# thanard/me-trpo

Measured on AMD Instinct MI355X. Metric: imagined env-steps/sec (KxBxH) over the full TRPO iteration, higher is better.
Workload: dtype f32

## Files before the change

### me-trpo_amd/_lib.py

```python
import ctypes as C
import os

import torch

_HERE = os.path.dirname(os.path.abspath(__file__))
LIB_PATH = os.path.join(_HERE, "libmetrpo.so")
MAX_LAYERS = 6

ENV_IDS = {'swimmer': 0, 'half_cheetah': 1, 'half-cheetah': 1, 'ant': 2, 'humanoid': 3, 'hopper': 4, 'snake': 5}
SAM_MODES = {'step_rand': 0, 'eps_rand': 1, 'model_mean_std': 2, 'model_mean': 3, 'model_med': 4, 'one_model': 5}
DYN_PRECISIONS = {'f32': 0, 'bf16': 1}
ACTS = {'identity': 0, 'tf.identity': 0, 'relu': 1, 'tf.nn.relu': 1, 'tanh': 2, 'tf.nn.tanh': 2, 'tf.tanh': 2}


class Dims(C.Structure):
    _fields_ = [('env', C.c_int32), ('ns', C.c_int32), ('na', C.c_int32), ('n_models', C.c_int32),
                ('dyn_n_hidden', C.c_int32), ('dyn_hidden', C.c_int32 * MAX_LAYERS), ('dyn_act', C.c_int32 * MAX_LAYERS),
                ('n_drop', C.c_int32), ('pol_n_hidden', C.c_int32), ('pol_hidden', C.c_int32 * MAX_LAYERS)]


class RolloutArgs(C.Structure):
    _fields_ = [('B', C.c_int32), ('T', C.c_int32), ('H', C.c_int32), ('sam_mode', C.c_int32), ('determ', C.c_int32),
                ('eval_all_heads', C.c_int32), ('d_pool', C.c_void_p), ('n_pool', C.c_int32), ('seed', C.c_uint64),
                ('stream_offset', C.c_uint64), ('d_eps', C.c_void_p), ('d_model_idx', C.c_void_p),
# ... 132 lines not shown
    'metrpo_bptt_grad_stochastic': (_I, [_P, _P, _I, _I, _D, _P, C.c_uint64, _P, _P, _P, _P]),
    'metrpo_set_exclusive': (_I, [_P, _I]),
    'metrpo_set_option': (_I, [_P, C.c_char_p, C.c_char_p]),
    'metrpo_get_option': (_I, [_P, C.c_char_p, C.c_char_p, _I]),
    'metrpo_option_name': (C.c_char_p, [_I]),
    'metrpo_last_rollout_kernel': (_I, [_P]),
    'metrpo_rollout_note': (C.c_char_p, [_P]),
    'metrpo_set_dyn_precision': (_I, [_P, _I]),
    'metrpo_get_dyn_precision': (_I, [_P]),
    'metrpo_policy_adam_reset': (_I, [_P, _P]),
    'metrpo_policy_adam_step': (_I, [_P, _P, _D, _D, _D, _D, _D, _P]),
    'metrpo_lbfgs_begin': (_I, [_P, _I, _P, C.POINTER(LbfgsOpts), _P, _P]),
    'metrpo_lbfgs_iterate': (_I, [_P, _P, _P, _P, _P, _P]),
    'metrpo_lbfgs_get_result': (_I, [_P, C.POINTER(LbfgsResult), _P]),
    'metrpo_lbfgs_policy': (_I, [_P, _P, _I, _I, _D, C.POINTER(LbfgsOpts), C.POINTER(LbfgsResult), _P]),
    'metrpo_get_dyn_adam': (_I, [_P, _P, _P, C.POINTER(_L), _P]),
    'metrpo_set_dyn_adam': (_I, [_P, _P, _P, _L, _P]),
    'metrpo_get_policy_adam': (_I, [_P, _P, _P, C.POINTER(_L), _P]),
    'metrpo_set_policy_adam': (_I, [_P, _P, _P, _L, _P]),
}
EXTRA_SYMBOLS = {
    'metrpo_rollout_generic': (_I, [_P, C.POINTER(RolloutArgs), _P]),
    'metrpo_has_mfma_path': (_I, [_P]),
    'metrpo_set_update_path': (_I, [_P, _I]),
    'metrpo_update_path': (_I, [_P, _L]),
    'metrpo_set_rollout_variant': (_I, [_P, _I]),
    'metrpo_set_det_path': (_I, [_P, _I]),
    'metrpo_probe_peaks': (_I, [_P, _P, _P]),
    'metrpo_schedulable_cus': (_I, [_P, _P]),
    'metrpo_debug_fvp_us': (_I, [_P, _P, _P]),
    'metrpo_debug_last_update': (_I, [_P, _P]),
    'metrpo_debug_persist_stats': (_I, [_P, _P, _I, _P]),
    'metrpo_debug_ws_retired': (_I, [_P, _P, _I]),
}


def load():
    if not os.path.exists(LIB_PATH):
        raise ImportError("libmetrpo.so not found at %s -- build it with `python -c 'import __graft_entry__ as g; "
                          "g.build()'` (hipcc --offload-arch=gfx950); there is no CPU fallback" % LIB_PATH)
    lib = C.CDLL(LIB_PATH)
    for table in (SYMBOLS, EXTRA_SYMBOLS):
        for name, (res, args) in table.items():
            fn = getattr(lib, name)
            fn.restype, fn.argtypes = res, args
    if lib.metrpo_abi_version() != 4:
        raise ImportError("libmetrpo.so ABI version mismatch")
    return lib


lib = load()


class MetrpoError(RuntimeError):
    pass


def check(rc, ctx=None):
    if rc != 0:
        msg = lib.metrpo_status_string(rc).decode()
        if ctx:
            msg += ": " + lib.metrpo_last_error(ctx).decode()
        raise MetrpoError(msg)
```

### me-trpo_amd/csrc/metrpo_internal.h

```cpp
#pragma once
#include <hip/hip_runtime.h>
#include <stdint.h>
#include <string>
#include <atomic>
#include <utility>
#include <vector>
#include "metrpo.h"
#include "xchg_device.h"

#define MAXL (METRPO_MAX_LAYERS + 1)
#define WAVE 64

struct NetDesc {
    int n_layers;
    int dims[MAXL + 1];
    int act[MAXL];
    int w_off[MAXL];
    int b_off[MAXL];
    int n_params;
    int api_w_off[MAXL];
    int api_b_off[MAXL];
    int api_n_params;
    int max_width;
};
// ... 48 lines not shown
    int rollout_variant = 0;
    DevBuf<float> d_partials;
    DevBuf<double> d_cg;
    DevBuf<float> d_vf;
    DevBuf<float> d_theta_try;
    DevBuf<double> d_valbuf;
    DevBuf<double> d_vbuf;
    DevBuf<double> d_gae_part;
    DevBuf<double> d_gram_part;
    DevBuf<unsigned int> d_ticket;
    DevBuf<float> d_hcache;
    DevBuf<void> d_sub;
    DevBuf<void> d_merr; DevBuf<double> d_merr_part;
    DevBuf<double> d_ppo_kl;
    DevBuf<void> d_mig; int mig_epoch = 0;
    void* nccl_comm = nullptr; int comm_world = 0, comm_rank = 0;
    void* xg_region = nullptr; void* xg_peer[XCHG_MAX_WORLD] = {}; int xg_world = 0, xg_rank = 0, xg_cap = 0; unsigned int xg_seq = 0; unsigned long long xg_timeout = 0;
    int pol_path = 1;
    DevBuf<void> d_pg; long long pg_fwd_rows = -1; const float* pg_fwd_obs = nullptr;
    int pol_f3 = 0;
    DevBuf<void> d_f3; long long f3_rows = -1; const float* f3_obs = nullptr; const float* f3_theta = nullptr; int f3_img_ok = 0;
    DevBuf<void> d_adam;
    long long adam_t = 0;
    DevBuf<void> d_train;
    DevBuf<double> d_train_part;
    DevBuf<void> d_big;
    DevBuf<void> d_res; unsigned int res_seq = 0;
    DevBuf<unsigned long long> d_skp_stats; int skp_stats_n = 0;
    std::vector<int> skp_tab_host;
    DevBuf<void> d_skp_tab; long long skp_key[8] = {-1, -1, -1, -1, -1, -1, -1, -1}; int skp_Jx[8] = {}, skp_Jmax = 0, skp_L = 0, skp_NSL = 0; int persist_failed = 0;
    int res_failed = 0;
    int last_ract_kernel = -1;
    DevBuf<int32_t> d_ract_model;
    int last_rollout_kernel = -1;
    int dyn_precision = METRPO_DYN_F32;
    DevBuf<uint16_t> d_dyn_bf16;
    double* h_upd = nullptr; unsigned long long upd_stamp = 0;
    DevBuf<double> d_lb; int lb_n = 0, lb_m = 0, lb_open = 0; double* h_lb = nullptr; unsigned long long lb_stamp = 0;
    int upd_pending = 0, upd_spec = 0, upd_changed_in_end = 0; metrpo_batch upd_batch = {}; metrpo_trpo_params upd_params = {}; metrpo_trpo_diag upd_diag = {};
    hipStream_t side_stream[METRPO_MAX_PAR_ROUNDS - 1] = {}; hipEvent_t ev_fork = nullptr, ev_join[METRPO_MAX_PAR_ROUNDS - 1] = {}; int side_ready = 0;
    double* h_pinned = nullptr;
    int n_sm = 256;
    int upd_tiles_per_wave = 1;
    int n_cu_sched = 0;
    int exclusive = 1;
    std::string opt_val[OPT_COUNT]; bool opt_set[OPT_COUNT] = {};
    hipEvent_t fvp_ev[32] = {}; int fvp_ev_n = 0, fvp_ev_made = 0;
    struct UpdLast { int family = -1, op = -1, table = -1, pt = 0, nrows = 0, splits = 0, kchunk = 0; } upd_last;
    std::string rollout_note;
    int fallback_logged = 0;
    std::vector<std::pair<void*, size_t>> ws_retired; size_t ws_retired_bytes = 0;
    std::string err;
};

constexpr size_t WS_RETIRED_MAX = (size_t)4 << 30;
static inline void ws_sweep(metrpo_ctx* c) {
    for (const auto& r : c->ws_retired) (void)hipFree(r.first);
    c->ws_retired.clear(); c->ws_retired_bytes = 0;
}
int set_err(metrpo_ctx* c, int code, const std::string& msg);
template <class T> static inline int ws_grow(metrpo_ctx* c, DevBuf<T>& b, size_t bytes, bool* grew = nullptr) {
    if (grew) *grew = false;
    if (bytes <= b.bytes) return METRPO_OK;
    if (b.p) {
        c->ws_retired.emplace_back((void*)b.p, b.bytes); c->ws_retired_bytes += b.bytes;
        b.p = nullptr; b.bytes = 0;
// ... 225 lines not shown
```

### me-trpo_amd/csrc/rollout_coop.hip

```cpp
#define COOP_MAIN_TU 1
#include "rollout_coop_kernel.h"

#define CENTRY_ENV(ENVID) CENTRY(ENVID, 5), CENTRY(ENVID, 4), CENTRY(ENVID, 3), CENTRY(ENVID, 2), CENTRY(ENVID, 1)
static const CoopEntry kCoop[] = {
    CENTRY_ENV(METRPO_ENV_SWIMMER), CENTRY_ENV(METRPO_ENV_HALF_CHEETAH), CENTRY_ENV(METRPO_ENV_HOPPER),
    CENTRY_ENV(METRPO_ENV_SNAKE), CENTRY_ENV(METRPO_ENV_ANT),
};
extern const CoopEntry kCoopK6[5], kCoopK7[5], kCoopK8[5], kCoopK9[5], kCoopK10[5];
constexpr int N_COOP = (int)(sizeof(kCoop) / sizeof(kCoop[0]));
static const CoopEntry& coop_entry(int idx) {
    if (idx < N_COOP) return kCoop[idx];
    const CoopEntry* wide[5] = {kCoopK6, kCoopK7, kCoopK8, kCoopK9, kCoopK10};
    return wide[(idx - N_COOP) / 5][(idx - N_COOP) % 5];
}

int coop_select_config(metrpo_ctx* c) {
    const ProblemDesc& pd = c->pd;
    if (mfma_shape_config(c) < 0 || pd.dyn.dims[1] != 64 || pd.dyn.dims[2] != 64 || pd.pol.dims[1] != 32 || pd.pol.dims[2] != 32) return -1;
    for (int i = 0; i < N_COOP + 25; ++i)
        if (coop_entry(i).env == pd.env && coop_entry(i).K == pd.K && coop_entry(i).kern[1][0] != nullptr) return i;
    return -1;
}

__global__ void __launch_bounds__(256) k_pad_dyn(NetDesc src, NetDesc dst, int K, const float* __restrict__ s, float* __restrict__ d) {
    const long long idx = (long long)blockIdx.x * 256 + threadIdx.x;
    if (idx >= (long long)K * dst.n_params) return;
    const int k = (int)(idx / dst.n_params), o = (int)(idx % dst.n_params);
    const float* sk = s + (size_t)k * src.n_params;
    float v = 0.0f;
    for (int l = 0; l < dst.n_layers; ++l) {
        const int din = dst.dims[l], dout = dst.dims[l + 1];
        if (o >= dst.w_off[l] && o < dst.w_off[l] + din * dout) {
            const int i = (o - dst.w_off[l]) / dout, j = (o - dst.w_off[l]) % dout;
            if (i < src.dims[l] && j < src.dims[l + 1]) v = sk[src.w_off[l] + i * src.dims[l + 1] + j];
        } else if (o >= dst.b_off[l] && o < dst.b_off[l] + dout) {
            const int j = o - dst.b_off[l];
            if (j < src.dims[l + 1]) v = sk[src.b_off[l] + j];
        }
    }
    d[idx] = v;
}

int launch_pad_dyn(metrpo_ctx* c, hipStream_t st) {
    const long long n = (long long)c->pd.K * c->dyn_pad.n_params;
    hipLaunchKernelGGL(k_pad_dyn, dim3((unsigned)((n + 255) / 256)), dim3(256), 0, st, c->pd.dyn, c->dyn_pad, c->pd.K, c->d_dyn.p, c->d_dyn_pad.p);
    HIP_TRY(c, hipGetLastError());
    return METRPO_OK;
}

int launch_rollout_coop(metrpo_ctx* c, int idx, const RolloutK& r_in, hipStream_t st, bool padded) {
    const CoopEntry& en = coop_entry(idx);
    const size_t sh = sizeof(float) * (size_t)en.lds_floats;
    const int tiles = (r_in.B + 15) / 16;
    RolloutK r = r_in;
    const int n_cu = (tiles > c->n_sm / 2) ? sched_cus(c, st) : c->n_sm;
    bool one = tiles <= n_cu || en.always_one;
    if (!one) {
        const long long slots = 2LL * n_cu, rounds = tiles / slots, rest = tiles % slots;
        const double t_one = (double)tiles / n_cu;
        const double t_two = en.pair * rounds + (rest == 0 ? 0.0 : rest <= n_cu ? 1.0 + en.rem_slope * (en.pair - 1.0) * rest / n_cu : en.pair);
        one = t_one < t_two;
    }
    if (c->rollout_variant == 2) one = false;
    if (one && tiles > n_cu && !ctx_exclusive(c)) one = false;
    if (!one && en.kern[0][0] == nullptr) return METRPO_EUNSUPPORTED;
    const int grid = one ? (tiles < n_cu ? tiles : n_cu) : tiles;
    if (one && tiles > grid) {
        const int ns = c->pd.ns;
        const size_t tile_bytes = sizeof(int32_t) * (1 + 32 + 16 * (size_t)ns);
        bool grew = false;
        { const int rc = ws_grow(c, c->d_mig, tile_bytes * (size_t)tiles, &grew); if (rc) return rc; }
        if (grew) { HIP_TRY(c, hipMemsetAsync(c->d_mig.p, 0, c->d_mig.bytes, st)); c->mig_epoch = 0; }
        const size_t cap = c->d_mig.bytes / tile_bytes;
        int32_t* base = (int32_t*)c->d_mig.p;
        r.mig_flag = base; r.mig_ts = base + cap; r.mig_model = base + 17 * cap;
        r.mig_obs = (float*)(base + 33 * cap);
        r.mig_epoch = ++c->mig_epoch;
        r.mig_err = comm_err_cell(c) + 1;
    }
    const bool draws = r.eps || r.model_idx || r.sel_noise || r.reset_idx || r.reset_model;
    const coop_kernel_t kern = en.kern[one ? 1 : 0][draws ? 1 : 0];
    if (sh > 64 * 1024) HIP_TRY(c, hipFuncSetAttribute((const void*)kern, hipFuncAttributeMaxDynamicSharedMemorySize, (int)sh));
    const float* dyn = c->d_dyn.p;
    if (padded) { const int rc = launch_pad_dyn(c, st); if (rc) return rc; dyn = c->d_dyn_pad.p; }
    hipLaunchKernelGGL(kern, dim3(grid), dim3(256), sh, st, r, dyn, c->d_theta.p, c->d_norm.p);
    HIP_TRY(c, hipGetLastError());
    return METRPO_OK;
}
```

### me-trpo_amd/csrc/rollout_coop_kernel.h

```cpp
#pragma once
#include "dyn_head_mfma.h"

#if defined(COOP_TIMING) && defined(COOP_MAIN_TU)
__device__ unsigned long long g_coop_phase[4][16];
#define PH_NOW() __builtin_readcyclecounter()
#define PH_DECL unsigned long long ph_t = PH_NOW(); unsigned long long ph_acc[14] = {0, 0, 0, 0, 0, 0, 0, 0, 0, 0, 0, 0, 0, 0};
#define PH_MARK(i) { if ((COOP_TIMING >> (i)) & 1) { const unsigned long long n_ = PH_NOW(); ph_acc[i] += n_ - ph_t; ph_t = n_; } }
#define PH_DUMP { if (lane == 0 && blockIdx.x == 0) for (int i_ = 0; i_ < 14; ++i_) g_coop_phase[wave][i_] = ph_acc[i_]; }
extern "C" int32_t metrpo_debug_coop_phases(unsigned long long* out) { return hipMemcpyFromSymbol(out, HIP_SYMBOL(g_coop_phase), sizeof(unsigned long long) * 64) == hipSuccess ? 0 : -1; }
#else
#define PH_DECL
#define PH_MARK(i)
#define PH_DUMP
#endif

#ifndef COOP_SKIP
#define COOP_SKIP 0
#endif
template <int ENV, int K>
struct Coop {
    using C = Cfg<ENV, 64, 32>;
    static constexpr int NS = C::NS, NA = C::NA, NSP = C::NSP;
    static constexpr int P0KS = 4 * C::OUT_CB;
    static constexpr int NPF = P0KS * 2 + 16 + 8;
    static constexpr int WV = ((16 * NSP + 16 * NS + 16 * NA + 3) / 4) * 4;
    static constexpr int O_BD0 = 4 * WV, O_BD1 = O_BD0 + K * 64, O_BD2 = O_BD1 + K * 64, O_BP0 = O_BD2 + K * NSP,
                         O_BP1 = O_BP0 + 32, O_BP2 = O_BP1 + 32, O_PW = O_BP2 + 16, O_H0 = O_PW + NPF * 64,
                         O_PART = O_H0 + K * 1024, O_RNG = O_PART + K * 4 * 16 * NSP, O_WX = O_RNG + 2 * 16 * 20,
                         O_AK = O_WX + 3 * ((K + 2) / 3) * C::NIN_KS * 64, TOTAL = O_AK + 2 * 16 * NA;
};

template <int ENV, int K, bool ONE, bool DRAWS>
__global__ void __launch_bounds__(256, ONE ? 1 : 2) k_rollout_coop(RolloutK r, const float* __restrict__ dynp,
                                                      const float* __restrict__ theta, const float* __restrict__ norm) {
    using L = Coop<ENV, K>;
    using C = typename L::C;
    constexpr int NS = C::NS, NA = C::NA, NSP = C::NSP, DH = 64, PH = 32, OUT_CB = C::OUT_CB;
    extern __shared__ __attribute__((aligned(16))) float lds[];
    const int tid = threadIdx.x, lane = tid & 63, wave = tid >> 6;
    const int e = lane & 15, q = lane >> 4;
    if (r.stop != nullptr && *r.stop != 0) return;
    int c_first = blockIdx.x, c_last = blockIdx.x, s_first = 0, e_last = r.T;
    if (ONE) {
        const long long total = (long long)((r.B + 15) / 16) * r.T;
        const long long Q = (total + gridDim.x - 1) / gridDim.x;
        const long long lo = (long long)blockIdx.x * Q, hi = (lo + Q < total) ? lo + Q : total;
        if (lo >= hi) return;
        c_first = (int)(lo / r.T); s_first = (int)(lo % r.T); c_last = (int)((hi - 1) / r.T); e_last = (int)((hi - 1) % r.T) + 1;
    }
    const int npc = c_last - c_first + 1;
    int b0 = 0, b = 0;
    bool active = false;
    uint64_t genv = 0;
    float* ST = lds + wave * L::WV;  float* NX = ST + 16 * NSP;
    float* ACT = lds + 16 * NSP + 16 * NS;

    float* BD0 = lds + L::O_BD0; float* BD1 = lds + L::O_BD1; float* BD2 = lds + L::O_BD2;
    float* BP0 = lds + L::O_BP0; float* BP1 = lds + L::O_BP1; float* BP2 = lds + L::O_BP2;
    float* PW = lds + L::O_PW; float* H0 = lds + L::O_H0; float* PART = lds + L::O_PART;
// ... 461 lines not shown
            for (int i = lane; i < lim; i += 64) r.mig_obs[(size_t)b0 * NS + i] = ST[(i / NS) * NSP + i % NS];
            if (q == 0) { r.mig_ts[b] = ts; r.mig_model[b] = cur_model; }
            __builtin_amdgcn_fence(__ATOMIC_RELEASE, "agent");
            if (lane == 0) __hip_atomic_store(&r.mig_flag[tile], r.mig_epoch, __ATOMIC_RELEASE, __HIP_MEMORY_SCOPE_AGENT);
        }
    } else {
        if (wave == 0 && r.last_obs != nullptr) {
            const int lim = min(16, r.B - b0) * NS;
            for (int i = lane; i < lim; i += 64) r.last_obs[(size_t)b0 * NS + i] = ST[(i / NS) * NSP + i % NS];
        }
        if (wave == 0 && q == 0 && active) {
            if (r.last_ts != nullptr) r.last_ts[b] = ts;
            if (r.last_model != nullptr) r.last_model[b] = cur_model;
        }
    }
    __syncthreads();
    }
    PH_DUMP
}


typedef void (*coop_kernel_t)(RolloutK, const float*, const float*, const float*);
template <int ENV> static constexpr bool coop_two_per_cu_spills() { return EnvDim<ENV>::NS > 16; }
struct CoopEntry { int env, K; coop_kernel_t kern[2][2]; int lds_floats; bool always_one; double pair, rem_slope; };
#define CENTRY(ENVID, KK) {ENVID, KK, {{k_rollout_coop<ENVID, KK, false, false>, k_rollout_coop<ENVID, KK, false, true>}, \
                                       {k_rollout_coop<ENVID, KK, true, false>, k_rollout_coop<ENVID, KK, true, true>}}, Coop<ENVID, KK>::TOTAL, coop_two_per_cu_spills<ENVID>(), \
                                       (ENVID == METRPO_ENV_SWIMMER) ? 1.50 : (ENVID == METRPO_ENV_SNAKE) ? 1.58 : 1.65, (ENVID == METRPO_ENV_SWIMMER) ? 0.0 : 1.0}
template <int ENV, int K, bool DRAWS> constexpr coop_kernel_t coop_one_kernel() {
    if constexpr (Coop<ENV, K>::TOTAL * sizeof(float) <= 160 * 1024) return k_rollout_coop<ENV, K, true, DRAWS>; else return nullptr;
}
#define CENTRY_ONE(ENVID, KK) {ENVID, KK, {{nullptr, nullptr}, {coop_one_kernel<ENVID, KK, false>(), coop_one_kernel<ENVID, KK, true>()}}, Coop<ENVID, KK>::TOTAL, true, 0.0, 0.0}
#define COOP_WIDE_TABLE(NAME, KK) extern const CoopEntry NAME[5]; const CoopEntry NAME[5] = { CENTRY_ONE(METRPO_ENV_SWIMMER, KK), CENTRY_ONE(METRPO_ENV_HALF_CHEETAH, KK), \
    CENTRY_ONE(METRPO_ENV_HOPPER, KK), CENTRY_ONE(METRPO_ENV_SNAKE, KK), CENTRY_ONE(METRPO_ENV_ANT, KK) };
```

### me-trpo_amd/engine.py

```python
import ctypes as C
from collections import namedtuple

import numpy as np
import torch

from . import _lib
from ._lib import lib, check

METRPO_UNSET = -100

Trajectory = namedtuple('Trajectory', 'obs act rew mean done tpath last_obs B T H')
"""Time-major device tensors of one rollout: obs [T,B,ns], act [T,B,na] (unclipped), rew [T,B],
mean [T,B,na], done [T,B] uint8, tpath [T,B] int32, last_obs [B,ns]."""


def _ptr(t):
    return C.c_void_p(t.data_ptr()) if t is not None else C.c_void_p(0)


def _f32(t, dev, shape=None):
    if t is None:
        return None
    t = torch.as_tensor(t, device=dev).to(torch.float32).contiguous()
    if shape is not None:
# ... 303 lines not shown
            assert tuple(r_obs.shape) == (B, self.ns) and r_ts.numel() == B and r_model.numel() == B
            a.d_init_obs, a.d_init_ts, a.d_init_model = r_obs.data_ptr(), r_ts.data_ptr(), r_model.data_ptr()
        if last_state is not None:
            assert all(t.dtype == torch.int32 and t.numel() == B for t in last_state)
            a.d_last_ts, a.d_last_model = last_state[0].data_ptr(), last_state[1].data_ptr()
        if stop is not None:
            assert stop.dtype == torch.int32
            a.d_stop = stop.data_ptr()
        if stop_batch:
            assert stop_cum is not None and stop_cum.dtype == torch.float64 and stop_cum.is_cuda
            a.stop_batch, a.d_stop_cum = int(stop_batch), stop_cum.data_ptr()
        fn = lib.metrpo_rollout_generic if force_generic else lib.metrpo_rollout
        self._chk(fn(self._ctx, C.byref(a), self._stream()))
        self._keep = (pool, eps, model_idx, sel_noise, reset_idx, reset_model, resume, last_state, stop, stop_cum)
        if no_draws and not chunked and not force_generic:
            self._ra_cache = ((id(out), pool.data_ptr(), B, T, H, sam_mode, bool(determ), bool(eval_all_heads), int(stream_offset)), a, out, pool)
        return out

    def sampler_progress(self, done, tpath, t0, batch_size, counts, state, stop):
        T, B = done.shape
        assert counts.dtype == torch.float64 and counts.numel() >= T and state.dtype == torch.float64 and stop.dtype == torch.int32
        self._chk(lib.metrpo_sampler_progress(self._ctx, _ptr(done), _ptr(tpath), int(T), int(B), int(t0), int(batch_size),
                                              _ptr(counts), _ptr(state), _ptr(stop), self._stream()))

    def rollout_path(self):
        if self.dyn_precision == 'bf16':
            return 7
        return int(lib.metrpo_set_rollout_variant(self._ctx, int(getattr(self, '_variant', 0))))

    def last_rollout_kernel(self):
        k = int(lib.metrpo_last_rollout_kernel(self._ctx))
        return {0: 'generic', 1: 'mfma-head-per-wave', 2: 'mfma-cooperative', 3: 'gemm-stepwise', 4: 'resident', 5: 'gemm-streamk', 6: 'streamk-persistent', 7: 'gemm-bf16'}.get(k)

    def rollout_note(self):
        return lib.metrpo_rollout_note(self._ctx).decode()

    def alloc_trajectory(self, B, T, H):
        dev, f = self.device, torch.float32
        return Trajectory(torch.empty(T, B, self.ns, dtype=f, device=dev), torch.empty(T, B, self.na, dtype=f, device=dev),
                          torch.empty(T, B, dtype=f, device=dev), torch.empty(T, B, self.na, dtype=f, device=dev),
                          torch.empty(T, B, dtype=torch.uint8, device=dev), torch.empty(T, B, dtype=torch.int32, device=dev),
                          torch.empty(B, self.ns, dtype=f, device=dev), B, T, H)

    def validation_cost(self, s0, T, gamma):
        s0 = _f32(s0, self.device); assert s0.shape[1] == self.ns
        costs = torch.empty(self.K, dtype=torch.float64, device=self.device)
        self._chk(lib.metrpo_validation_cost(self._ctx, _ptr(s0), s0.shape[0], int(T), float(gamma), _ptr(costs), self._stream()))
        return costs

    def gae(self, traj, coeffs, gamma, lam, stats=None):
        dev = self.device
        T, B = traj.T, traj.B
        adv = torch.empty(T, B, dtype=torch.float32, device=dev); ret = torch.empty_like(adv)
        valid = torch.empty(T, B, dtype=torch.uint8, device=dev)
        if stats is None:
            stats = torch.zeros(3, dtype=torch.float64, device=dev)
        if coeffs is not None:
            if isinstance(coeffs, torch.Tensor) and coeffs.is_cuda:
                coeffs = coeffs.to(torch.float64).contiguous()
            else:
                F = 2 * self.ns + 4
                if getattr(self, '_coef_pin', None) is None:
                    self._coef_pin = [torch.empty(F, dtype=torch.float64).pin_memory() for _ in range(2)]
                    self._coef_dev = [torch.empty(F, dtype=torch.float64, device=dev) for _ in range(2)]
                    self._coef_i = 0
                self._coef_i ^= 1
# ... 393 lines not shown
```

Baseline: 1.948 billion.

## Split cooperative rollout heads across two wave groups in 512-thread blocks

Adds a head-split variant of the cooperative MFMA rollout kernel that runs 8 waves per block. The dynamics-model heads are divided between two groups of four waves: group 0 also carries the policy, RNG and reward waves, while group 1 takes the remaining heads plus a helper that computes extra layer-0 work. This is on by default for swimmer, hopper and snake with K from 2 to 5 on the one-block path. The aim is more per-CU parallelism and a shorter per-step critical path, at the cost of more LDS, more registers per block and a larger barrier across 512 threads.

```diff
diff --git a/me-trpo_amd/_lib.py b/me-trpo_amd/_lib.py
--- a/me-trpo_amd/_lib.py
+++ b/me-trpo_amd/_lib.py
@@ -188,6 +188,8 @@
     'metrpo_debug_last_update': (_I, [_P, _P]),
     'metrpo_debug_persist_stats': (_I, [_P, _P, _I, _P]),
     'metrpo_debug_ws_retired': (_I, [_P, _P, _I]),
+    'metrpo_debug_coop_waves': (_I, [_P]),
+    'metrpo_set_coop_split': (_I, [_P, _I]),
 }
 
 
diff --git a/me-trpo_amd/csrc/metrpo_internal.h b/me-trpo_amd/csrc/metrpo_internal.h
--- a/me-trpo_amd/csrc/metrpo_internal.h
+++ b/me-trpo_amd/csrc/metrpo_internal.h
@@ -104,6 +104,8 @@
     int res_failed = 0;
     int last_ract_kernel = -1;
     DevBuf<int32_t> d_ract_model;
+    int coop_no_split = 0;
+    int last_coop_waves = 0;
     int last_rollout_kernel = -1;
     int dyn_precision = METRPO_DYN_F32;
     DevBuf<uint16_t> d_dyn_bf16;
diff --git a/me-trpo_amd/csrc/rollout_coop.hip b/me-trpo_amd/csrc/rollout_coop.hip
--- a/me-trpo_amd/csrc/rollout_coop.hip
+++ b/me-trpo_amd/csrc/rollout_coop.hip
@@ -6,6 +6,11 @@
     CENTRY_ENV(METRPO_ENV_SWIMMER), CENTRY_ENV(METRPO_ENV_HALF_CHEETAH), CENTRY_ENV(METRPO_ENV_HOPPER),
     CENTRY_ENV(METRPO_ENV_SNAKE), CENTRY_ENV(METRPO_ENV_ANT),
 };
+static const CoopSplitEntry kCoopSplit[] = { CSPLIT_ENV(METRPO_ENV_SWIMMER), CSPLIT_ENV(METRPO_ENV_HOPPER), CSPLIT_ENV(METRPO_ENV_SNAKE) };
+static const CoopSplitEntry* coop_split_entry(int env, int K) {
+    for (const CoopSplitEntry& s : kCoopSplit) if (s.env == env && s.K == K) return &s;
+    return nullptr;
+}
 extern const CoopEntry kCoopK6[5], kCoopK7[5], kCoopK8[5], kCoopK9[5], kCoopK10[5];
 constexpr int N_COOP = (int)(sizeof(kCoop) / sizeof(kCoop[0]));
 static const CoopEntry& coop_entry(int idx) {
@@ -50,7 +55,6 @@
 
 int launch_rollout_coop(metrpo_ctx* c, int idx, const RolloutK& r_in, hipStream_t st, bool padded) {
     const CoopEntry& en = coop_entry(idx);
-    const size_t sh = sizeof(float) * (size_t)en.lds_floats;
     const int tiles = (r_in.B + 15) / 16;
     RolloutK r = r_in;
     const int n_cu = (tiles > c->n_sm / 2) ? sched_cus(c, st) : c->n_sm;
@@ -79,11 +83,16 @@
         r.mig_err = comm_err_cell(c) + 1;
     }
     const bool draws = r.eps || r.model_idx || r.sel_noise || r.reset_idx || r.reset_model;
-    const coop_kernel_t kern = en.kern[one ? 1 : 0][draws ? 1 : 0];
+    const CoopSplitEntry* sp = (one && !c->coop_no_split) ? coop_split_entry(en.env, en.K) : nullptr;
+    const coop_kernel_t kern = sp ? sp->kern[draws ? 1 : 0] : en.kern[one ? 1 : 0][draws ? 1 : 0];
+    const size_t sh = sizeof(float) * (size_t)(sp ? sp->lds_floats : en.lds_floats);
     if (sh > 64 * 1024) HIP_TRY(c, hipFuncSetAttribute((const void*)kern, hipFuncAttributeMaxDynamicSharedMemorySize, (int)sh));
     const float* dyn = c->d_dyn.p;
     if (padded) { const int rc = launch_pad_dyn(c, st); if (rc) return rc; dyn = c->d_dyn_pad.p; }
-    hipLaunchKernelGGL(kern, dim3(grid), dim3(256), sh, st, r, dyn, c->d_theta.p, c->d_norm.p);
+    hipLaunchKernelGGL(kern, dim3(grid), dim3(sp ? 512 : 256), sh, st, r, dyn, c->d_theta.p, c->d_norm.p);
     HIP_TRY(c, hipGetLastError());
+    c->last_coop_waves = sp ? 8 : 4;
     return METRPO_OK;
 }
+extern "C" int32_t metrpo_debug_coop_waves(const metrpo_ctx* c) { return c ? c->last_coop_waves : METRPO_ENULL; }
+extern "C" int32_t metrpo_set_coop_split(metrpo_ctx* c, int32_t split) { if (!c) return METRPO_ENULL; c->coop_no_split = split ? 0 : 1; return METRPO_OK; }
diff --git a/me-trpo_amd/csrc/rollout_coop_kernel.h b/me-trpo_amd/csrc/rollout_coop_kernel.h
--- a/me-trpo_amd/csrc/rollout_coop_kernel.h
+++ b/me-trpo_amd/csrc/rollout_coop_kernel.h
@@ -2,12 +2,12 @@
 #include "dyn_head_mfma.h"
 
 #if defined(COOP_TIMING) && defined(COOP_MAIN_TU)
-__device__ unsigned long long g_coop_phase[4][16];
+__device__ unsigned long long g_coop_phase[8][16];
 #define PH_NOW() __builtin_readcyclecounter()
 #define PH_DECL unsigned long long ph_t = PH_NOW(); unsigned long long ph_acc[14] = {0, 0, 0, 0, 0, 0, 0, 0, 0, 0, 0, 0, 0, 0};
 #define PH_MARK(i) { if ((COOP_TIMING >> (i)) & 1) { const unsigned long long n_ = PH_NOW(); ph_acc[i] += n_ - ph_t; ph_t = n_; } }
 #define PH_DUMP { if (lane == 0 && blockIdx.x == 0) for (int i_ = 0; i_ < 14; ++i_) g_coop_phase[wave][i_] = ph_acc[i_]; }
-extern "C" int32_t metrpo_debug_coop_phases(unsigned long long* out) { return hipMemcpyFromSymbol(out, HIP_SYMBOL(g_coop_phase), sizeof(unsigned long long) * 64) == hipSuccess ? 0 : -1; }
+extern "C" int32_t metrpo_debug_coop_phases(unsigned long long* out) { return hipMemcpyFromSymbol(out, HIP_SYMBOL(g_coop_phase), sizeof(unsigned long long) * 128) == hipSuccess ? 0 : -1; }
 #else
 #define PH_DECL
 #define PH_MARK(i)
@@ -17,14 +17,14 @@
 #ifndef COOP_SKIP
 #define COOP_SKIP 0
 #endif
-template <int ENV, int K>
+template <int ENV, int K, int NWV = 4>
 struct Coop {
     using C = Cfg<ENV, 64, 32>;
     static constexpr int NS = C::NS, NA = C::NA, NSP = C::NSP;
     static constexpr int P0KS = 4 * C::OUT_CB;
     static constexpr int NPF = P0KS * 2 + 16 + 8;
     static constexpr int WV = ((16 * NSP + 16 * NS + 16 * NA + 3) / 4) * 4;
-    static constexpr int O_BD0 = 4 * WV, O_BD1 = O_BD0 + K * 64, O_BD2 = O_BD1 + K * 64, O_BP0 = O_BD2 + K * NSP,
+    static constexpr int O_BD0 = NWV * WV, O_BD1 = O_BD0 + K * 64, O_BD2 = O_BD1 + K * 64, O_BP0 = O_BD2 + K * NSP,
                          O_BP1 = O_BP0 + 32, O_BP2 = O_BP1 + 32, O_PW = O_BP2 + 16, O_H0 = O_PW + NPF * 64,
                          O_PART = O_H0 + K * 1024, O_RNG = O_PART + K * 4 * 16 * NSP, O_WX = O_RNG + 2 * 16 * 20,
                          O_AK = O_WX + 3 * ((K + 2) / 3) * C::NIN_KS * 64, TOTAL = O_AK + 2 * 16 * NA;
@@ -552,3 +552,469 @@
 #define CENTRY_ONE(ENVID, KK) {ENVID, KK, {{nullptr, nullptr}, {coop_one_kernel<ENVID, KK, false>(), coop_one_kernel<ENVID, KK, true>()}}, Coop<ENVID, KK>::TOTAL, true, 0.0, 0.0}
 #define COOP_WIDE_TABLE(NAME, KK) extern const CoopEntry NAME[5]; const CoopEntry NAME[5] = { CENTRY_ONE(METRPO_ENV_SWIMMER, KK), CENTRY_ONE(METRPO_ENV_HALF_CHEETAH, KK), \
     CENTRY_ONE(METRPO_ENV_HOPPER, KK), CENTRY_ONE(METRPO_ENV_SNAKE, KK), CENTRY_ONE(METRPO_ENV_ANT, KK) };
+
+template <int ENV, int K, bool DRAWS, int G>
+__device__ __forceinline__ void coop_split_body(const RolloutK& r, const float* __restrict__ dynp, const float* __restrict__ theta,
+                                                const float* __restrict__ norm, float* lds, const int w) {
+    using L = Coop<ENV, K, 8>;
+    using C = typename L::C;
+    static_assert(C::OUT_CB == 1 && K >= 2 && K <= 5, "head-split form: one output col-block, 2 ... 5 heads");
+    constexpr int NS = C::NS, NA = C::NA, NSP = C::NSP, DH = 64, PH = 32;
+    constexpr int KG = (G == 0) ? K / 2 : K - K / 2, K0 = (G == 0) ? 0 : K / 2;
+    constexpr int KX = (G == 1) ? K / 2 : 0;
+    const int tid = threadIdx.x, lane = tid & 63, wave = 4 * G + w;
+    const int e = lane & 15, q = lane >> 4;
+    const bool pol = (G == 0 && w == 0), rngw = (G == 0 && w == 1), reww = (G == 0 && w == 2), helper = (G == 1 && w == 0);
+    if (r.stop != nullptr && *r.stop != 0) return;
+    const long long total = (long long)((r.B + 15) / 16) * r.T;
+    const long long Q = (total + gridDim.x - 1) / gridDim.x;
+    const long long lo = (long long)blockIdx.x * Q, hi = (lo + Q < total) ? lo + Q : total;
+    if (lo >= hi) return;
+    const int c_first = (int)(lo / r.T), s_first = (int)(lo % r.T), c_last = (int)((hi - 1) / r.T), e_last = (int)((hi - 1) % r.T) + 1;
+    const int npc = c_last - c_first + 1;
+    int b0 = 0, b = 0;
+    bool active = false;
+    uint64_t genv = 0;
+    float* ST = lds + wave * L::WV;  float* NX = ST + 16 * NSP;
+    float* ACT = lds + 16 * NSP + 16 * NS;
+    float* BD0 = lds + L::O_BD0; float* BD1 = lds + L::O_BD1; float* BD2 = lds + L::O_BD2;
+    float* BP0 = lds + L::O_BP0; float* BP1 = lds + L::O_BP1; float* BP2 = lds + L::O_BP2;
+    float* PW = lds + L::O_PW; float* H0 = lds + L::O_H0; float* PART = lds + L::O_PART;
+    float* AK = lds + L::O_AK;
+    float* RNGB = lds + L::O_RNG;
+
+    float wd0[KG][C::NIN_KS], wd1[KG][16], wd2[KG][4];
+#pragma unroll
+    for (int k = 0; k < KG; ++k) {
+        const float* __restrict__ pk = dynp + (size_t)(K0 + k) * C::PD;
+#pragma unroll
+        for (int s = 0; s < C::NIN_KS; ++s) { const int i = 4 * s + q; wd0[k][s] = (i < C::NIN) ? pk[C::dW0 + i * DH + 16 * w + e] : 0.0f; }
+#pragma unroll
+        for (int kk = 0; kk < 16; ++kk) { const int i = chained_in(kk, q); wd1[k][kk] = pk[C::dW1 + i * DH + 16 * w + e]; }
+#pragma unroll
+        for (int rr = 0; rr < 4; ++rr) { const int i = 16 * w + 4 * q + rr; wd2[k][rr] = (e < NS) ? pk[C::dW2 + i * NS + e] : 0.0f; }
+    }
+    float wx0[KX > 0 ? KX : 1][C::NIN_KS];
+#pragma unroll
+    for (int j = 0; j < KX; ++j) {
+        const float* __restrict__ pk = dynp + (size_t)j * C::PD;
+#pragma unroll
+        for (int s = 0; s < C::NIN_KS; ++s) { const int i = 4 * s + q; wx0[j][s] = (i < C::NIN && helper) ? pk[C::dW0 + i * DH + e] : 0.0f; }
+    }
+    for (int i = tid; i < K * 64; i += 512) { const int k = i >> 6, u = i & 63; BD0[i] = dynp[(size_t)k * C::PD + C::db0 + u]; BD1[i] = dynp[(size_t)k * C::PD + C::db1 + u]; }
+    for (int i = tid; i < K * NSP; i += 512) { const int k = i / NSP, u = i % NSP; BD2[i] = (u < NS) ? dynp[(size_t)k * C::PD + C::db2 + u] : 0.0f; }
+    if (tid < 32) { BP0[tid] = theta[C::pb0 + tid]; BP1[tid] = theta[C::pb1 + tid]; }
+    if (tid < 16) BP2[tid] = (tid < NA) ? theta[C::pb2 + tid] : 0.0f;
+    for (int i = tid; i < L::NPF * 64; i += 512) {
+        const int f = i >> 6, ln = i & 63, ee = ln & 15, qq = ln >> 4;
+        float wv = 0.0f;
+        if (f < L::P0KS * 2) { const int j = f >> 1, cb = f & 1, in = chained_in(j, qq); wv = (in < NS) ? theta[C::pW0 + in * PH + 16 * cb + ee] : 0.0f; }
+        else if (f < L::P0KS * 2 + 16) { const int g = f - L::P0KS * 2, kk = g >> 1, cb = g & 1, in = chained_in(kk, qq); wv = theta[C::pW1 + in * PH + 16 * cb + ee]; }
+        else { const int kk = f - L::P0KS * 2 - 16, in = chained_in(kk, qq); wv = (ee < NA) ? theta[C::pW2 + in * NA + ee] : 0.0f; }
+        PW[i] = wv;
+    }
+    float sig[4];
+#pragma unroll
+    for (int rr = 0; rr < 4; ++rr) sig[rr] = (4 * q + rr < NA) ? expf(fmaxf(theta[C::pLS + 4 * q + rr], LOG_MIN_STD)) : 0.0f;
+    DynInNorm<C> in;
+    DynOutNorm<C> out;
+    in.load(norm, q);
+    out.load(norm, q);
+    auto step_draws = [&](int tt, uint4& ds, float (&zz)[4]) {
+        ds = rng_draw(r.seed, genv, tt, RNG_STEP, 0);
+        const uint4 b0k = (q == 0) ? ds : ((NA > 4) ? rng_draw(r.seed, genv, tt, RNG_STEP, 2 * q) : ds);
+        normal2(b0k.x, b0k.y, zz[0], zz[1]);
+        if (NA > 2) { const uint4 b1k = rng_draw(r.seed, genv, tt, RNG_STEP, 2 * q + 1); normal2(b1k.x, b1k.y, zz[2], zz[3]); }
+    };
+    constexpr bool LOCAL_REWARD = (ENV == METRPO_ENV_SWIMMER || ENV == METRPO_ENV_SNAKE);
+    constexpr int RDIM = (ENV == METRPO_ENV_SWIMMER) ? 5 : 7;
+    constexpr int NPR = (G == 0) ? 1 : 0;
+    float w0r[NPR ? L::P0KS * 2 : 1], w1r[NPR ? 16 : 1], w2r[NPR ? 8 : 1];
+    f32x4 bp0r[2], bp1r[2], bp2r;
+    __syncthreads();
+    if (G == 0) {
+        const float* pw0 = PW + lane, *pw1 = PW + L::P0KS * 2 * 64 + lane, *pw2 = PW + (L::P0KS * 2 + 16) * 64 + lane;
+#pragma unroll
+        for (int f = 0; f < L::P0KS * 2; ++f) w0r[NPR ? f : 0] = pw0[f * 64];
+#pragma unroll
+        for (int f = 0; f < 16; ++f) w1r[NPR ? f : 0] = pw1[f * 64];
+#pragma unroll
+        for (int f = 0; f < 8; ++f) w2r[NPR ? f : 0] = pw2[f * 64];
+        bp0r[0] = *(const f32x4*)&BP0[4 * q]; bp0r[1] = *(const f32x4*)&BP0[16 + 4 * q];
+        bp1r[0] = *(const f32x4*)&BP1[4 * q]; bp1r[1] = *(const f32x4*)&BP1[16 + 4 * q];
+        bp2r = *(const f32x4*)&BP2[4 * q];
+    }
+    PH_DECL
+    for (int pc = 0; pc < npc; ++pc) {
+    const int tile = (pc == npc - 1) ? c_first : (pc == 0 ? c_last : c_first + pc);
+    const int t_begin = (tile == c_first) ? s_first : 0, t_end = (tile == c_last) ? e_last : r.T;
+    b0 = tile * 16; b = b0 + e; active = b < r.B; genv = r.stream_offset + (uint64_t)b;
+    const bool resume = r.init_obs != nullptr;
+    int cur_model = 0, ts = 0;
+    if (t_begin > 0) {
+        if (tid == 0) {
+            unsigned long long t0 = 0; int spins = 0;
+            while (__hip_atomic_load(&r.mig_flag[tile], __ATOMIC_ACQUIRE, __HIP_MEMORY_SCOPE_AGENT) != r.mig_epoch) {
+                __builtin_amdgcn_s_sleep(4);
+                if (++spins == 4096) t0 = wall_clock64();
+                if (spins > 4096 && (spins & 1023) == 0 && wall_clock64() - t0 > 200000000ull) { if (r.mig_err) *r.mig_err = 1.0; break; }
+            }
+        }
+        __syncthreads();
+        __builtin_amdgcn_fence(__ATOMIC_ACQUIRE, "agent");
+        cur_model = r.mig_model[b]; ts = r.mig_ts[b];
+#pragma unroll
+        for (int rr = 0; rr < 4; ++rr) {
+            const int dim = 4 * q + rr;
+            ST[e * NSP + dim] = (dim < NS) ? r.mig_obs[(size_t)b * NS + dim] : 0.0f;
+        }
+    } else {
+        int row = 0;
+        if (active && !resume) {
+            const uint4 d0 = rng_draw(r.seed, genv, 0, RNG_RESET, 0);
+            row = (DRAWS && r.reset_idx != nullptr) ? r.reset_idx[b] : rng_index(d0.x, r.n_pool);
+            cur_model = (DRAWS && r.reset_model != nullptr) ? r.reset_model[b] : rng_index(d0.y, K);
+        }
+        if (active && resume) { cur_model = r.init_model[b]; ts = r.init_ts[b]; }
+#pragma unroll
+        for (int rr = 0; rr < 4; ++rr) {
+            const int dim = 4 * q + rr;
+            ST[e * NSP + dim] = (dim < NS) ? (resume ? r.init_obs[(size_t)(active ? b : 0) * NS + dim] : r.pool[(size_t)row * NS + dim]) : 0.0f;
+        }
+    }
+    __syncthreads();
+
+    f32x4 xc;
+#pragma unroll
+    for (int rr = 0; rr < 4; ++rr) xc[rr] = ST[e * NSP + 4 * q + rr];
+    uint4 dstep = make_uint4(0, 0, 0, 0); float z[4] = {0.f, 0.f, 0.f, 0.f};
+    step_draws(r.t0 + t_begin, dstep, z);
+    __builtin_amdgcn_s_waitcnt(0x0F70);
+    for (int t = t_begin; t < t_end; ++t) {
+        PH_MARK(9)
+        const size_t trow = (size_t)t * r.B;
+        const unsigned ub = (unsigned)b;
+        constexpr int KS_STATE = (NS - C::NDROP) / 4;
+        f32x4 h0[KG], hx0[KX > 0 ? KX : 1];
+        if (!pol) {
+#pragma unroll
+            for (int k = 0; k < KG; ++k) h0[k] = *(const f32x4*)&BD0[(K0 + k) * 64 + 16 * w + 4 * q];
+#pragma unroll
+            for (int j = 0; j < KX; ++j) hx0[j] = *(const f32x4*)&BD0[j * 64 + 4 * q];
+#pragma unroll
+            for (int s = 0; s < KS_STATE; ++s) {
+                const float x = in.get_state(ST, NSP, e, s);
+#pragma unroll
+                for (int k = 0; k < KG; ++k) h0[k] = MFMA16(wd0[k][s], x, h0[k]);
+                if (helper) {
+#pragma unroll
+                    for (int j = 0; j < KX; ++j) hx0[j] = MFMA16(wx0[j][s], x, hx0[j]);
+                }
+            }
+        }
+        if (rngw) {
+            uint4 dn; float zn[4] = {0.f, 0.f, 0.f, 0.f};
+            step_draws(r.t0 + t + 1, dn, zn);
+            float* dst = RNGB + (((t + 1) & 1) * 16 + e) * 20;
+            if (q == 0) *(uint4*)dst = dn;
+            *(float4*)(dst + 4 + 4 * q) = make_float4(zn[0], zn[1], zn[2], zn[3]);
+        }
+        if constexpr (G == 0) {
+        if (pol) {
+            f32x4 p0[2], p1[2];
+            f32x4 m0, m1 = {0.f, 0.f, 0.f, 0.f};
+            {
+                p0[0] = bp0r[0]; p0[1] = bp0r[1];
+#pragma unroll
+                for (int j = 0; j < L::P0KS; ++j) {
+                    p0[0] = MFMA16(w0r[2 * j], xc[j & 3], p0[0]);
+                    p0[1] = MFMA16(w0r[2 * j + 1], xc[j & 3], p0[1]);
+                }
+            }
+            {
+                p1[0] = bp1r[0]; p1[1] = bp1r[1]; m0 = bp2r;
+#pragma unroll
+                for (int kk = 0; kk < 8; ++kk) {
+                    const float hv = tanh_fast(p0[kk >> 2][kk & 3]);
+                    p1[0] = MFMA16(w1r[2 * kk], hv, p1[0]);
+                    p1[1] = MFMA16(w1r[2 * kk + 1], hv, p1[1]);
+                }
+#pragma unroll
+                for (int kk = 0; kk < 8; kk += 2) {
+                    const float ha = tanh_fast(p1[kk >> 2][kk & 3]);
+                    m0 = MFMA16(w2r[kk], ha, m0);
+                    const float hb = tanh_fast(p1[(kk + 1) >> 2][(kk + 1) & 3]);
+                    m1 = MFMA16(w2r[kk + 1], hb, m1);
+                }
+                __builtin_amdgcn_sched_group_barrier(0x100, 64, 0);
+                __builtin_amdgcn_sched_group_barrier(0x008, L::P0KS * 2, 0);
+                __builtin_amdgcn_sched_group_barrier(0x402, 5, 0);
+#pragma unroll
+                for (int kk = 0; kk < 8; ++kk) {
+                    __builtin_amdgcn_sched_group_barrier(0x008, 1, 0);
+                    __builtin_amdgcn_sched_group_barrier(0x402, 3, 0);
+                    __builtin_amdgcn_sched_group_barrier(0x008, 1, 0);
+                    __builtin_amdgcn_sched_group_barrier(0x402, 2, 0);
+                }
+#pragma unroll
+                for (int kk = 0; kk < 8; ++kk) {
+                    __builtin_amdgcn_sched_group_barrier(0x008, 1, 0);
+                    if (kk < 7) __builtin_amdgcn_sched_group_barrier(0x402, 5, 0);
+                }
+            }
+            const f32x4 mu = m0 + m1;
+            PH_MARK(0)
+#pragma unroll
+            for (int rr = 0; rr < 4; ++rr) {
+                const int d = 4 * q + rr;
+                if (d < NA) {
+                    float a = mu[rr];
+                    if (!r.determ) {
+                        const float zz = (DRAWS && r.eps != nullptr) ? (active ? (r.eps + trow * NA)[ub * NA + d] : 0.0f) : z[rr];
+                        a = fmaf(zz, sig[rr], a);
+                    }
+                    AK[e * NA + d] = a; AK[16 * NA + e * NA + d] = mu[rr];
+                    const float ac = fminf(fmaxf(a, -1.0f), 1.0f);
+                    ACT[e * NA + d] = ac;
+                }
+            }
+        }
+        }
+        __syncthreads();
+        PH_MARK(1)
+        if (!pol) {
+            float xin[C::NIN_KS];
+#pragma unroll
+            for (int s = KS_STATE; s < C::NIN_KS; ++s) xin[s] = in.get(ST, NSP, ACT, e, s);
+#pragma unroll
+            for (int s = KS_STATE; s < C::NIN_KS; ++s) {
+#pragma unroll
+                for (int k = 0; k < KG; ++k) h0[k] = MFMA16(wd0[k][s], xin[s], h0[k]);
+                if (helper) {
+#pragma unroll
+                    for (int j = 0; j < KX; ++j) hx0[j] = MFMA16(wx0[j][s], xin[s], hx0[j]);
+                }
+            }
+#pragma unroll
+            for (int k = 0; k < KG; ++k) {
+#pragma unroll
+                for (int rr = 0; rr < 4; ++rr) h0[k][rr] = relu1(h0[k][rr]);
+                *(f32x4*)&H0[(K0 + k) * 1024 + w * 256 + q * 64 + e * 4] = h0[k];
+            }
+            if (helper) {
+#pragma unroll
+                for (int j = 0; j < KX; ++j) {
+#pragma unroll
+                    for (int rr = 0; rr < 4; ++rr) hx0[j][rr] = relu1(hx0[j][rr]);
+                    *(f32x4*)&H0[j * 1024 + q * 64 + e * 4] = hx0[j];
+                }
+            }
+        } else {
+            {
+                const size_t base_a = (trow + b0) * NA;
+                const int lim_a = min(16, r.B - b0) * NA;
+#pragma unroll
+                for (int j = 0; j < (16 * NA + 63) / 64; ++j) {
+                    const int i = lane + 64 * j;
+                    if (i < lim_a) { (r.act + base_a)[(unsigned)i] = AK[i]; (r.mean + base_a)[(unsigned)i] = AK[16 * NA + i]; }
+                }
+            }
+            const size_t base = (trow + b0) * NS;
+            const int lim = min(16, r.B - b0) * NS;
+            float ov[(16 * NS + 63) / 64];
+#pragma unroll
+            for (int j = 0; j < (16 * NS + 63) / 64; ++j) { const int i = min(lane + 64 * j, 16 * NS - 1); ov[j] = ST[(i / NS) * NSP + i % NS]; }
+#pragma unroll
+            for (int j = 0; j < (16 * NS + 63) / 64; ++j) { const int i = lane + 64 * j; if (i < lim) (r.obs + base)[(unsigned)i] = ov[j]; }
+        }
+        PH_MARK(2)
+        __syncthreads();
+        PH_MARK(3)
+        float su2 = 0.0f;
+        if constexpr (G == 0) {
+#pragma unroll
+            for (int d = 0; d < NA; ++d) { const float ac = ACT[e * NA + d]; su2 = fmaf(ac, ac, su2); }
+        }
+        PH_MARK(10)
+        __builtin_amdgcn_s_setprio(1);
+        f32x4 h1[KG];
+#pragma unroll
+        for (int k = 0; k < KG; ++k) h1[k] = *(const f32x4*)&BD1[(K0 + k) * 64 + 16 * w + 4 * q];
+        f32x4 hb[2][KG];
+#pragma unroll
+        for (int k = 0; k < KG; ++k) hb[0][k] = *(const f32x4*)&H0[(K0 + k) * 1024 + q * 64 + e * 4];
+#pragma unroll
+        for (int cb = 0; cb < 4; ++cb) {
+            if (cb < 3) {
+#pragma unroll
+                for (int k = 0; k < KG; ++k) hb[(cb + 1) % 2][k] = *(const f32x4*)&H0[(K0 + k) * 1024 + (cb + 1) * 256 + q * 64 + e * 4];
+            }
+#pragma unroll
+            for (int rr = 0; rr < 4; ++rr) {
+#pragma unroll
+                for (int k = 0; k < KG; ++k) h1[k] = MFMA16(wd1[k][cb * 4 + rr], hb[cb % 2][k][rr], h1[k]);
+                __builtin_amdgcn_sched_barrier(0x94);
+                pin_order(h1);
+            }
+        }
+        PH_MARK(11)
+#pragma unroll
+        for (int k = 0; k < KG; ++k)
+#pragma unroll
+            for (int rr = 0; rr < 4; ++rr) h1[k][rr] = relu1(h1[k][rr]);
+        __builtin_amdgcn_sched_barrier(0);
+        {
+            f32x4 po[KG];
+#pragma unroll
+            for (int k = 0; k < KG; ++k) po[k] = f32x4{0.f, 0.f, 0.f, 0.f};
+#pragma unroll
+            for (int rr = 0; rr < 4; ++rr)
+#pragma unroll
+                for (int k = 0; k < KG; ++k) po[k] = MFMA16(wd2[k][rr], h1[k][rr], po[k]);
+#pragma unroll
+            for (int k = 0; k < KG; ++k) *(f32x4*)&PART[(((K0 + k) * 4 + w) * 16 + e) * NSP + 4 * q] = po[k];
+        }
+        __builtin_amdgcn_s_setprio(0);
+        PH_MARK(4)
+        __syncthreads();
+        PH_MARK(5)
+        ts += 1;
+        int sel = cur_model;
+        if (r.sam_mode == METRPO_SAM_STEP_RAND) sel = (DRAWS && r.model_idx != nullptr) ? (active ? (r.model_idx + trow)[ub] : 0) : rng_index(dstep.z, K);
+        if (r.sam_mode == METRPO_SAM_ONE_MODEL) sel = 0;
+        const bool simple = (r.sam_mode == METRPO_SAM_STEP_RAND || r.sam_mode == METRPO_SAM_EPS_RAND || r.sam_mode == METRPO_SAM_ONE_MODEL);
+        f32x4 nx;
+        {
+            const int off = e * NSP + 4 * q;
+            const f32x4 sv = xc;
+            auto head = [&](int k) -> f32x4 {
+                const float* pp = PART + (size_t)k * 4 * 16 * NSP + off;
+                f32x4 o = *(const f32x4*)&BD2[k * NSP + 4 * q];
+                o += (*(const f32x4*)&pp[0] + *(const f32x4*)&pp[16 * NSP]) + (*(const f32x4*)&pp[2 * 16 * NSP] + *(const f32x4*)&pp[3 * 16 * NSP]);
+                return out.apply(0, o, sv);
+            };
+            if (simple) nx = head(sel);
+            else {
+                f32x4 hv[K], m = {0.f, 0.f, 0.f, 0.f};
+#pragma unroll
+                for (int k = 0; k < K; ++k) { hv[k] = head(k); m += hv[k]; }
+                m /= (float)K;
+                if (r.sam_mode == METRPO_SAM_MODEL_MEAN) nx = m;
+                else if (r.sam_mode == METRPO_SAM_MODEL_MEAN_STD) {
+                    f32x4 var = {0.f, 0.f, 0.f, 0.f};
+#pragma unroll
+                    for (int k = 0; k < K; ++k) { const f32x4 d = hv[k] - m; var += d * d; }
+                    float zz[4] = {0.f, 0.f, 0.f, 0.f};
+                    if (!DRAWS || r.sel_noise == nullptr) normal4(rng_draw(r.seed, genv, r.t0 + t, RNG_SELNOISE, q), zz);
+#pragma unroll
+                    for (int rr = 0; rr < 4; ++rr) {
+                        const int dim = 4 * q + rr;
+                        const float nz = (DRAWS && r.sel_noise != nullptr) ? ((active && dim < NS) ? (r.sel_noise + trow * NS)[ub * NS + dim] : 0.0f) : zz[rr];
+                        nx[rr] = fmaf(nz, sqrtf(var[rr] / (float)K), m[rr]);
+                    }
+                } else {
+                    constexpr int r_lo = (K - 1) / 2, r_hi = K / 2;
+                    f32x4 lo4 = {0.f, 0.f, 0.f, 0.f}, hi4 = lo4;
+#pragma unroll
+                    for (int k = 0; k < K; ++k) {
+                        int rank[4] = {0, 0, 0, 0};
+#pragma unroll
+                        for (int j = 0; j < K; ++j)
+#pragma unroll
+                            for (int rr = 0; rr < 4; ++rr) rank[rr] += (hv[j][rr] < hv[k][rr]) || (hv[j][rr] == hv[k][rr] && j < k);
+#pragma unroll
+                        for (int rr = 0; rr < 4; ++rr) { if (rank[rr] == r_lo) lo4[rr] = hv[k][rr]; if (rank[rr] == r_hi) hi4[rr] = hv[k][rr]; }
+                    }
+                    nx = (lo4 + hi4) * 0.5f;
+                }
+            }
+        }
+        PH_MARK(6)
+        bool dn = false;
+        if constexpr (G == 0) {
+            float cost = 0.0f;
+            if (LOCAL_REWARD) {
+                const float xr = nx[RDIM & 3];
+                if (ENV == METRPO_ENV_SWIMMER) cost = -(xr - 1e-2f * (su2 / (float)NA));
+                else cost = -(xr - 1e-2f * 0.5f * su2);
+                dn = (ts >= r.H);
+                if (reww && q == ((RDIM & 15) >> 2) && active) { (r.rew + trow)[ub] = -cost; (r.done + trow)[ub] = dn ? 1 : 0; (r.tpath + trow)[ub] = ts - 1; }
+            } else {
+                float pen = 0.0f;
+#pragma unroll
+                for (int rr = 0; rr < 4; ++rr) {
+                    const int dim = 4 * q + rr;
+                    if (dim < NS) {
+                        NX[e * NS + dim] = nx[rr];
+                        if (ENV == METRPO_ENV_HOPPER && dim >= 2) pen += fmaxf(fabsf(nx[rr]) - 100.0f, 0.0f);
+                    }
+                }
+                wave_lds_sync();
+                const float* xn = NX + e * NS;
+                pen = xor_sum(pen);
+                cost = -(xn[5] - 0.01f * 0.5f * su2 - 10.0f * fmaxf(0.45f - xn[0], 0.0f) - 10.0f * fmaxf(fabsf(xn[1]) - 0.2f, 0.0f) - pen);
+                dn = dn || (ts >= r.H);
+                if (reww && q == 0 && active) { (r.rew + trow)[ub] = -cost; (r.done + trow)[ub] = dn ? 1 : 0; (r.tpath + trow)[ub] = ts - 1; }
+            }
+        } else dn = (ts >= r.H);
+        PH_MARK(7)
+        if (__any(dn)) {
+            int row = 0;
+            if (dn) {
+                if (active) {
+                    row = (DRAWS && r.reset_idx != nullptr) ? (r.reset_idx + trow + r.B)[ub] : rng_index(dstep.w, r.n_pool);
+                    cur_model = (DRAWS && r.reset_model != nullptr) ? (r.reset_model + trow + r.B)[ub] : rng_index16(dstep.z, K);
+                }
+                ts = 0;
+            }
+#pragma unroll
+            for (int rr = 0; rr < 4; ++rr) {
+                const int dim = 4 * q + rr;
+                if (dim < NS) { const float xv = dn ? r.pool[(unsigned)(row * NS + dim)] : nx[rr]; ST[e * NSP + dim] = xv; xc[rr] = xv; }
+            }
+        } else {
+            xc = nx;
+            *(f32x4*)&ST[e * NSP + 4 * q] = nx;
+        }
+        {
+            const float* src = RNGB + (((t + 1) & 1) * 16 + e) * 20;
+            dstep = *(const uint4*)src;
+            if (G == 0) { const float4 zf = *(const float4*)(src + 4 + 4 * q); z[0] = zf.x; z[1] = zf.y; z[2] = zf.z; z[3] = zf.w; }
+        }
+        wave_lds_sync();
+        PH_MARK(8)
+    }
+    if (t_end < r.T) {
+        if (pol) {
+            const int lim = 16 * NS;
+            for (int i = lane; i < lim; i += 64) r.mig_obs[(size_t)b0 * NS + i] = ST[(i / NS) * NSP + i % NS];
+            if (q == 0) { r.mig_ts[b] = ts; r.mig_model[b] = cur_model; }
+            __builtin_amdgcn_fence(__ATOMIC_RELEASE, "agent");
+            if (lane == 0) __hip_atomic_store(&r.mig_flag[tile], r.mig_epoch, __ATOMIC_RELEASE, __HIP_MEMORY_SCOPE_AGENT);
+        }
+    } else {
+        if (pol && r.last_obs != nullptr) {
+            const int lim = min(16, r.B - b0) * NS;
+            for (int i = lane; i < lim; i += 64) r.last_obs[(size_t)b0 * NS + i] = ST[(i / NS) * NSP + i % NS];
+        }
+        if (pol && q == 0 && active) {
+            if (r.last_ts != nullptr) r.last_ts[b] = ts;
+            if (r.last_model != nullptr) r.last_model[b] = cur_model;
+        }
+    }
+    __syncthreads();
+    }
+    PH_DUMP
+}
+
+template <int ENV, int K, bool DRAWS>
+__global__ void __launch_bounds__(512, 1) k_rollout_coop_split(RolloutK r, const float* __restrict__ dynp,
+                                                                const float* __restrict__ theta, const float* __restrict__ norm) {
+    extern __shared__ __attribute__((aligned(16))) float lds[];
+    const int wave = __builtin_amdgcn_readfirstlane((int)(threadIdx.x >> 6));
+    if (wave < 4) coop_split_body<ENV, K, DRAWS, 0>(r, dynp, theta, norm, lds, wave);
+    else coop_split_body<ENV, K, DRAWS, 1>(r, dynp, theta, norm, lds, wave - 4);
+}
+struct CoopSplitEntry { int env, K; coop_kernel_t kern[2]; int lds_floats; };
+#define CSPLIT(ENVID, KK) {ENVID, KK, {k_rollout_coop_split<ENVID, KK, false>, k_rollout_coop_split<ENVID, KK, true>}, Coop<ENVID, KK, 8>::TOTAL}
+#define CSPLIT_ENV(ENVID) CSPLIT(ENVID, 5), CSPLIT(ENVID, 4), CSPLIT(ENVID, 3), CSPLIT(ENVID, 2)
diff --git a/me-trpo_amd/engine.py b/me-trpo_amd/engine.py
--- a/me-trpo_amd/engine.py
+++ b/me-trpo_amd/engine.py
@@ -359,6 +359,12 @@
         k = int(lib.metrpo_last_rollout_kernel(self._ctx))
         return {0: 'generic', 1: 'mfma-head-per-wave', 2: 'mfma-cooperative', 3: 'gemm-stepwise', 4: 'resident', 5: 'gemm-streamk', 6: 'streamk-persistent', 7: 'gemm-bf16'}.get(k)
 
+    def set_coop_split(self, split):
+        self._chk(lib.metrpo_set_coop_split(self._ctx, int(bool(split))))
+
+    def last_coop_waves(self):
+        return int(lib.metrpo_debug_coop_waves(self._ctx))
+
     def rollout_note(self):
         return lib.metrpo_rollout_note(self._ctx).decode()
 
```

Result: faster. 1.969 billion, median of 6 (+1.0%).
